# study-game-engines/directx-renderer-kurth

Measured on AMD Instinct MI355X. Metric: physics steps/sec at 100k rigid bodies, higher is better.
Workload: dtype f32; 1 GPU; c3: 100k mixed colliders (sphere/capsule/OBB), dt 1/120 s, 30 solver iterations; bodies=100000, broadphase_pairs=611032, manifolds=251275, contacts=317267, joints=0, recoveries=0, parallelism=1 gpu

## Files before the change

directx-renderer-kurth_amd/csrc/cluster.h:

```cpp
#pragma once
#include "world.h"

#define CL_TASKS_PER_PHASE 2u
#define CL_SUBCOUNTERS 8u
#define CL_LOCAL_STATIC 0xFFFFu
#define CL_SERIAL_COLOR 64u

MI_DEV u32 clHash(u32 x) { x ^= x >> 16; x *= 0x7feb352du; x ^= x >> 15; x *= 0x846ca68bu; x ^= x >> 16; return x; }
MI_DEV u32 clPhaseOffset(const u32* counters, u32 p)
{
	u32 off = p ? counters[CTR_CL_NUM_TASKS] : 0u;
	for (u32 q = CL_MAX_PHASES - 1u; q > p && p; --q) off += counters[CTR_CL_NUM_TASKS + q];
	return off;
}
struct ClTask
{
	u32 first, count, numBodies, numShared, numColors, serialStart, numRows, sharedBase;
	u32 colorStart[72];
};
static_assert(sizeof(ClTask) == 320, "task header");

bool cluster_color_setup(World& w, u32 computeUnits);
void cluster_color_launch(World& w, u32 nj);
u32 cluster_solve_setup(const World& w);
```

directx-renderer-kurth_amd/csrc/k_cluster_solve.hip:

```cpp
#include "cluster.h"
#include "solver_rows.h"
#include "joint_solve.h"

#define CL_MAX_LOCAL_TASKS 8u
#define CLS_LANES 512u
#define CLQ_QUADS (CLS_LANES / 4u)
#define CLQ_SETS 7u
#define CLQ_REG_CONTACTS (CLQ_QUADS * CLQ_SETS)
#define CLQ_SETS_JOINTS 4u
#define CL_SPIN_LIMIT (1u << 22)

typedef u32 u32x4 __attribute__((ext_vector_type(4)));

struct QuadRow { V3 dT, aT, dN, aN; float mT, mN, bias, friction, lamN, lamT; };
#define CLQ_ZERO_FLOAT4S (2u * CLQ_QUADS + 4u)
#define CLQ_ROW_FLOAT4S 14u

struct ClLocal
{
	u32 first, count, numBodies, numShared, numColors, serialStart, numContacts, phase, key, sharedBase, numJoints;
	u32 bodyOff;
	u32 infoOff;
	u32 regContacts, spill, rowOff, rowCap, scratchBase;
	u32 ldsColors;
	u32 colorStart[68];
};

struct ClArgs
{
	u32* counters; const ClTask* tasks; const u32* bodyList; const u32* phaseMask; const u32* sharedSlot;
	const u32* mKeySorted; const u32* mLocal; const u32* cEntry;
	const float4* rowPlanes; const float4* rowShared; float2* rowLambda; float4* rowScratch; u32 scratchContacts;
	u32 regContactsCap;
	u32 ldsRowsCap;
	u32 predictDiv, pollSleep;
	float4* vel; u64* flow; u64* trace;
	size_t rowCap; u32 nb, flowBytes, epoch, itBegin, itEnd, ldsFloat4s;
	const u32* jointClassStart; const uint2* taskJoints; const uint4* jointTable; float* jointUpd[MI_JOINT_TYPES]; const float4* invIw; u32 numJointClasses;
};

MI_DEV float clQuadSum(float p)
{
	float q = p + __builtin_bit_cast(float, __builtin_amdgcn_update_dpp(0, __builtin_bit_cast(int, p), 0xB1, 0xF, 0xF, false));
	return q + __builtin_bit_cast(float, __builtin_amdgcn_update_dpp(0, __builtin_bit_cast(int, q), 0x4E, 0xF, 0xF, false));
}
MI_DEV void clSolveQuad(QuadRow& r, V3& x)
{
	float vt = clQuadSum(rowDot3(x, r.dT));
	float maxFriction = r.friction * r.lamN;
	float newT = rowClampSym(__builtin_fmaf(-r.mT, vt, r.lamT), maxFriction);
	float d = newT - r.lamT; r.lamT = newT;
	x = rowFma(d, r.aT, x);
	float vn = clQuadSum(rowDot3(x, r.dN));
	float newN = fmaxf(__builtin_fmaf(-r.mN, vn - r.bias, r.lamN), 0.f);
	d = newN - r.lamN; r.lamN = newN;
	x = rowFma(d, r.aN, x);
}
MI_DEV void clBuildQuadRow(QuadRow& r, u32& addr, const ClLocal& L, const ClArgs& A, const float4* lds, u32 p, u32 q, u32 zeroRec, u32& slotOut, u32& kOut)
{
	const u32 e = A.cEntry[(size_t)4u * L.first + p], mp = e & 0xFFFu, k = e >> 12, slot = L.first + mp;
	const u32 ab = A.mLocal[slot], local = q < 2u ? (ab & 0xFFFFu) : (ab >> 16);
	const float4 sh = A.rowShared[slot];
	ContactRow row; loadRow(row, k, slot, A.rowCap, A.rowPlanes, A.rowLambda);
	const bool isStatic = local == CL_LOCAL_STATIC;
	addr = (isStatic ? zeroRec : L.bodyOff + 2u * local) + (q & 1u);
	const float invMass = isStatic ? 0.f : lds[L.bodyOff + 2u * local].w;
	const V3 t = v3(row.p0.x, row.p0.y, row.p0.z), n = v3(sh.x, sh.y, sh.z);
	if (q == 0u) { r.dT = -t; r.aT = -(invMass * t); r.dN = -n; r.aN = -(invMass * n); }
	else if (q == 1u) { r.dT = -v3(row.p0.w, row.p1.x, row.p1.y); r.aT = -v3(row.p3.w, row.p4.x, row.p4.y); r.dN = -v3(row.p2.y, row.p2.z, row.p2.w); r.aN = -v3(row.p5.y, row.p5.z, row.p5.w); }
	else if (q == 2u) { r.dT = t; r.aT = invMass * t; r.dN = n; r.aN = invMass * n; }
	else { r.dT = v3(row.p1.z, row.p1.w, row.p2.x); r.aT = v3(row.p4.z, row.p4.w, row.p5.x); r.dN = v3(row.p3.x, row.p3.y, row.p3.z); r.aN = v3(row.p6.x, row.p6.y, row.p6.z); }
	r.mT = row.p7.x; r.mN = row.p6.w; r.bias = row.p7.y; r.friction = sh.w; r.lamN = row.lam.x; r.lamT = row.lam.y;
	slotOut = slot; kOut = k;
}
template <typename T> MI_DEV T clLdsAt(const float4* lds, u32 byte) { return *(const T*)((const char*)lds + byte); }
template <typename PTR> MI_DEV void clStoreQuadRow(PTR P, u32 q, const QuadRow& r, u32 addr)
{
	P[3u * q] = make_float4(r.dT.x, r.dT.y, r.dT.z, r.aT.x); P[3u * q + 1u] = make_float4(r.aT.y, r.aT.z, r.dN.x, r.dN.y); P[3u * q + 2u] = make_float4(r.dN.z, r.aN.x, r.aN.y, r.aN.z);
	if (q == 0u) P[12] = make_float4(r.mT, r.mN, r.bias, r.friction);
	const u32 other = (u32)__builtin_amdgcn_update_dpp(0, (int)addr, 0xB1, 0xF, 0xF, false);
	const u32 otherPair = (u32)__builtin_amdgcn_update_dpp(0, (int)(addr | (other << 16)), 0x4E, 0xF, 0xF, false);
	if (q == 0u) P[13] = make_float4(r.lamN, r.lamT, __uint_as_float(addr | (other << 16)), __uint_as_float(otherPair));
}
MI_DEV u32 clPairAddr(u32 pair, u32 q) { return (q & 1u) ? (pair >> 16) : (pair & 0xFFFFu); }
#define CLQ_PAIR_WORD(q) (54u + ((q) >> 1))
template <typename PTR> MI_DEV void clLoadQuadRow(QuadRow& r, u32& addr, PTR P, u32 q)
{
	float4 a = P[3u * q], b = P[3u * q + 1u], c = P[3u * q + 2u], d = P[12], e = P[13];
	r.dT = v3f4(a); r.aT = v3(a.w, b.x, b.y); r.dN = v3(b.z, b.w, c.x); r.aN = v3(c.y, c.z, c.w);
	r.mT = d.x; r.mN = d.y; r.bias = d.z; r.friction = d.w; r.lamN = e.x; r.lamT = e.y;
	addr = clPairAddr(__float_as_uint(q < 2u ? e.z : e.w), q);
}

template <bool JOINTS> __global__ void __launch_bounds__(CLS_LANES) k_cl_solve(ClArgs A)
{
	extern __shared__ float4 lds[];
	__shared__ ClLocal sTask[CL_MAX_LOCAL_TASKS];
	__shared__ u32 sNumTasks, sAbort;
	__shared__ u32 sRegStart[CL_SERIAL_COLOR + 4u];
	const u32 tid = threadIdx.x, G = gridDim.x, quad = tid >> 2, q = tid & 3u;
	constexpr u32 SETS = JOINTS ? CLQ_SETS_JOINTS : CLQ_SETS;
	u32* status = A.counters + CTR_FLOW_STATUS;
	__amdgpu_buffer_rsrc_t rsrc = __builtin_amdgcn_make_buffer_rsrc(A.flow, 0, A.flowBytes, 0x00020000);
	const u32 zeroBase = A.ldsFloat4s - CLQ_ZERO_FLOAT4S, zeroRec = zeroBase + 2u * CLQ_QUADS, sinkRec = zeroRec + 2u;

	if (tid == 0)
	{
		if (A.trace) A.trace[(size_t)blockIdx.x * CL_TRACE_ROWS * CL_TRACE_WORDS + 15 * 32] = wall_clock64();
		u32 nT = 0, off = 0, used = 0;
		bool bad = A.counters[CTR_CL_STATUS] != 0u;
		for (u32 p = 0; p < CL_MAX_PHASES; ++p)
		{
			u32 tasksInPhase = A.counters[CTR_CL_NUM_TASKS + p];
			if (tasksInPhase > CL_TASKS_PER_PHASE * G) { bad = true; atomicOr(status, 128u); }
			off = clPhaseOffset(A.counters, p);
			u32 t = (blockIdx.x + G - (off % G)) % G;
			for (; t < tasksInPhase && !bad; t += G)
			{
				u32 key = p * CL_MAX_TASKS + t;
				const ClTask* T = A.tasks + key;
				const u32 tj = (A.jointClassStart && p == 0u) ? A.jointClassStart[(size_t)key * (CL_MAX_JOINT_CLASSES + 2u) + CL_MAX_JOINT_CLASSES] : 0u;
				if (!T->count && !tj) continue;
				if (nT == CL_MAX_LOCAL_TASKS) { bad = true; atomicOr(status, 256u); break; }
				ClLocal& L = sTask[nT];
				L.first = T->first; L.count = T->count; L.numBodies = T->numBodies; L.numShared = T->numShared; L.numColors = T->numColors; L.serialStart = T->serialStart; L.numContacts = T->numRows;
				L.phase = p; L.key = key; L.sharedBase = T->sharedBase; L.numJoints = tj;
				if (tj > CLS_LANES || (tj && nT)) { bad = true; atomicOr(status, 2048u); }
				for (u32 c = 0; c <= CL_SERIAL_COLOR + 1u; ++c) L.colorStart[c] = T->colorStart[c];
				L.colorStart[CL_SERIAL_COLOR + 2u] = L.colorStart[CL_SERIAL_COLOR + 1u]; L.colorStart[CL_SERIAL_COLOR + 3u] = L.colorStart[CL_SERIAL_COLOR + 1u];
				L.bodyOff = used; used += 2u * L.numBodies;
				L.infoOff = used * 4u; used += (3u * L.numBodies + 3u) / 4u;
				L.regContacts = (nT == 0) ? min(L.numContacts, min(CLQ_QUADS * SETS, A.regContactsCap)) : 0u;
				L.rowOff = 0; L.rowCap = 0; L.spill = 0;
				const u32 regBase = L.numContacts - L.regContacts;
				L.ldsColors = 0; while (L.ldsColors < L.numColors && L.colorStart[L.ldsColors + 1u] <= regBase) ++L.ldsColors;
				if (nT == 0) for (u32 c = 0; c < CL_SERIAL_COLOR + 4u; ++c) sRegStart[c] = L.colorStart[c] - regBase;
				++nT;
			}
		}
		if (used + CLQ_ZERO_FLOAT4S > A.ldsFloat4s) { bad = true; atomicOr(status, 512u); }
		u32 ldsRowsLeft = A.ldsRowsCap;
		for (u32 k = 0; k < nT && !bad; ++k)
		{
			ClLocal& L = sTask[k];
			u32 want = L.numContacts - L.regContacts;
			u32 left = A.ldsFloat4s - used - CLQ_ZERO_FLOAT4S;
			u32 fit = min(left / CLQ_ROW_FLOAT4S, ldsRowsLeft);
			u32 cap = want < fit ? want : fit;
			L.rowOff = used; L.rowCap = cap; used += CLQ_ROW_FLOAT4S * cap; ldsRowsLeft -= cap; L.scratchBase = 0; L.spill = want - cap;
			if (want > cap) { L.scratchBase = atomicAdd(&A.counters[CTR_CL_SCRATCH], want - cap); if (L.scratchBase + (want - cap) > A.scratchContacts) { bad = true; atomicOr(status, 1024u); break; } }
		}
		if (bad) atomicOr(status, 64u);
		sNumTasks = nT; sAbort = (bad || __hip_atomic_load(status, __ATOMIC_RELAXED, __HIP_MEMORY_SCOPE_AGENT) != 0u) ? 1u : 0u;
	}
	__syncthreads();
	if (sAbort) return;
	const u32 numTasks = sNumTasks;
	if (!numTasks) return;

	for (u32 k = 0; k < numTasks; ++k)
	{
		const ClLocal& L = sTask[k];
		u32* info = (u32*)lds + L.infoOff;
		for (u32 l = tid; l < L.numBodies; l += CLS_LANES)
		{
			u32 g = A.bodyList[(size_t)L.key * CL_BODY_STRIDE + l];
			u32 pm = A.phaseMask[g];
			u32 deg = __popc(pm), rank = __popc(pm & ((1u << L.phase) - 1u));
			u32 below = pm & ((1u << L.phase) - 1u);
			u32 prev = below ? 31u - (u32)__clz(below) : 31u - (u32)__clz(pm);
			info[3 * l] = g; info[3 * l + 1] = deg | (rank << 8);
			info[3 * l + 2] = (l < L.numShared) ? A.sharedSlot[(size_t)prev * (A.nb + 1u) + g] : 0u;
			lds[L.bodyOff + 2 * l] = A.vel[2 * g]; lds[L.bodyOff + 2 * l + 1] = A.vel[2 * g + 1];
		}
	}
	for (u32 i = tid; i < CLQ_ZERO_FLOAT4S; i += CLS_LANES) lds[zeroBase + i] = make_float4(0.f, 0.f, 0.f, 0.f);
	__syncthreads();
	QuadRow rows[SETS]; u32 addr[SETS];
	{
		const ClLocal& L = sTask[0];
		const u32 regBase = L.numContacts - L.regContacts;
#pragma unroll
		for (u32 s = 0; s < SETS; ++s)
		{
			const u32 p = s * CLQ_QUADS + quad;
			rows[s].dT = rows[s].aT = rows[s].dN = rows[s].aN = v3(0.f, 0.f, 0.f); rows[s].mT = rows[s].mN = rows[s].bias = rows[s].friction = rows[s].lamN = rows[s].lamT = 0.f; addr[s] = sinkRec;
			if (p < L.regContacts) { u32 slot, kk; clBuildQuadRow(rows[s], addr[s], L, A, lds, regBase + p, q, zeroBase + 2u * quad, slot, kk); }
		}
	}
	for (u32 k = 0; k < numTasks; ++k)
	{
		const ClLocal& L = sTask[k];
		for (u32 p = quad; p < L.numContacts - L.regContacts; p += CLQ_QUADS)
		{
			QuadRow r; u32 a, slot, kk;
			clBuildQuadRow(r, a, L, A, lds, p, q, zeroBase + 2u * quad, slot, kk);
			if (p >= L.spill) clStoreQuadRow(lds + L.rowOff + (p - L.spill) * CLQ_ROW_FLOAT4S, q, r, a);
			else clStoreQuadRow(A.rowScratch + (size_t)(L.scratchBase + p) * CLQ_ROW_FLOAT4S, q, r, a);
		}
	}
	u32 tailStart0 = sTask[0].numColors, tailSet = 0, myTail = 255u;
	{
		const ClLocal& L = sTask[0];
		const u32 regBase = L.numContacts - L.regContacts, endPos = L.colorStart[L.numColors];
		if (L.numColors && endPos > regBase)
		{
			const u32 blk = (endPos - regBase - 1u) >> 4;
			while (tailStart0 > 0u && L.colorStart[tailStart0 - 1u] >= regBase && ((L.colorStart[tailStart0 - 1u] - regBase) >> 4) == blk) --tailStart0;
			if (L.numColors - tailStart0 < 2u) tailStart0 = L.numColors;
			else
			{
				tailSet = (L.colorStart[tailStart0] - regBase) / CLQ_QUADS;
				const u32 p = regBase + tailSet * CLQ_QUADS + quad;
				if (p >= L.colorStart[tailStart0] && p < endPos) { myTail = tailStart0; while (L.colorStart[myTail + 1u] <= p) ++myTail; }
			}
		}
		tailStart0 = __builtin_amdgcn_readfirstlane(tailStart0); tailSet = __builtin_amdgcn_readfirstlane(tailSet);
	}
	const u32 bodyOff0 = sTask[0].bodyOff;
	u32 jClass = 0xFFFFFFFFu, jType = 0, jA = 0, jB = 0, jRdA = zeroRec, jWrA = sinkRec, jRdB = zeroRec, jWrB = sinkRec; float* jRec = nullptr;
	const u32 numJoints0 = (JOINTS && sTask[0].phase == 0u) ? sTask[0].numJoints : 0u;
	if (JOINTS && tid < numJoints0)
	{
		const u32* cs = A.jointClassStart + (size_t)sTask[0].key * (CL_MAX_JOINT_CLASSES + 2u);
		uint2 e = A.taskJoints[cs[CL_MAX_JOINT_CLASSES + 1u] + tid];
		uint4 t4 = A.jointTable[e.x];
		jType = t4.x & 0xFFu; jClass = t4.x >> 8; jA = t4.z; jB = t4.w;
		jRec = A.jointUpd[jType] + (size_t)t4.y * jointUpdateFloats(jType);
		u32 la = e.y & 0xFFFFu, lb = e.y >> 16;
		if (la != CL_LOCAL_STATIC) { jRdA = bodyOff0 + 2u * la; jWrA = jRdA; }
		if (lb != CL_LOCAL_STATIC) { jRdB = bodyOff0 + 2u * lb; jWrB = jRdB; }
	}
	__syncthreads();
	u64* trace = A.trace ? A.trace + (size_t)blockIdx.x * CL_TRACE_ROWS * CL_TRACE_WORDS : nullptr;
	if (trace && tid == 0)
	{
		trace[15 * 32 + 1] = wall_clock64();
		for (u32 k = 0; k < numTasks && k < 5u; ++k) { trace[15 * 32 + 2 + 4 * k] = sTask[k].count; trace[15 * 32 + 3 + 4 * k] = sTask[k].numColors; trace[15 * 32 + 4 + 4 * k] = sTask[k].numShared; trace[15 * 32 + 5 + 4 * k] = sTask[k].phase | (sTask[k].numBodies << 8) | ((u64)sTask[k].numContacts << 32); trace[15 * 32 + 22 + k] = sTask[k].rowCap | ((u64)sTask[k].regContacts << 32); trace[15 * 32 + 27 + k] = sTask[k].spill | ((u64)(k == 0u ? sTask[0].numColors - tailStart0 : 0u) << 32); }
	}

#define CLQ_SOLVE_SET(S_, CS_, END_) if ((S_) < SETS) { const u32 pos = (S_) * CLQ_QUADS + quad; if (pos >= (CS_) && pos < (END_)) { float4 b = lds[addr[(S_) < SETS ? (S_) : 0u]]; V3 x = v3f4(b); clSolveQuad(rows[(S_) < SETS ? (S_) : 0u], x); lds[addr[(S_) < SETS ? (S_) : 0u]] = make_float4(x.x, x.y, x.z, b.w); } }
#define CLQ_PREFETCH(POS_) { const u32 in_ = max((POS_), spill) + quad - spill; if (in_ < rowCap) pfW = ((const u32*)(lds + rowOff + in_ * CLQ_ROW_FLOAT4S))[CLQ_PAIR_WORD(q)]; }
#define CLQ_SOLVE_ROWS(CS_, END_) \
	{ \
		u32 w = pfW; \
		CLQ_PREFETCH(END_) \
		for (u32 p = (CS_) + quad; p < (END_); p += CLQ_QUADS) \
		{ \
			const bool inLds = p >= spill; \
			QuadRow r; u32 a; float4 b; \
			float4* P = lds + rowOff + (inLds ? p - spill : 0u) * CLQ_ROW_FLOAT4S; \
			float4* S = A.rowScratch + (size_t)(scratchBase + (inLds ? 0u : p)) * CLQ_ROW_FLOAT4S; \
			u32 wn = 0u; if (p + CLQ_QUADS < (END_) && p + CLQ_QUADS >= spill) wn = ((const u32*)(lds + rowOff + (p + CLQ_QUADS - spill) * CLQ_ROW_FLOAT4S))[CLQ_PAIR_WORD(q)]; \
			if (inLds) { u32 unused; a = clPairAddr(w, q); b = lds[a]; clLoadQuadRow(r, unused, P, q); } else { clLoadQuadRow(r, a, S, q); b = lds[a]; } \
			V3 x = v3f4(b); clSolveQuad(r, x); lds[a] = make_float4(x.x, x.y, x.z, b.w); \
			if (q == 0u) { if (inLds) ((float2*)(P + 13))[0] = make_float2(r.lamN, r.lamT); else ((float2*)(S + 13))[0] = make_float2(r.lamN, r.lamT); } \
			w = wn; \
		} \
	}
#define CLQ_SOLVE_ROWS_LDS(CS_, END_) \
	{ \
		const u32 i = (CS_) - spill + quad, endR = (END_) - spill, w = pfW; \
		pfW = clLdsAt<u32>(lds, __umul24(min(endR + quad, lastRow), CLQ_ROW_FLOAT4S * 16u) + pairByte); \
		if (i < endR) \
		{ \
			const u32 a = clPairAddr(w, q), rowByte = __umul24(i, CLQ_ROW_FLOAT4S * 16u) + rowsByte, own = rowByte + q * 48u; \
			const float4 b = lds[a], r0 = clLdsAt<float4>(lds, own), r1 = clLdsAt<float4>(lds, own + 16u), r2 = clLdsAt<float4>(lds, own + 32u), r3 = clLdsAt<float4>(lds, rowByte + 192u); \
			const float2 lam = clLdsAt<float2>(lds, rowByte + 208u); \
			QuadRow r; r.dT = v3f4(r0); r.aT = v3(r0.w, r1.x, r1.y); r.dN = v3(r1.z, r1.w, r2.x); r.aN = v3(r2.y, r2.z, r2.w); \
			r.mT = r3.x; r.mN = r3.y; r.bias = r3.z; r.friction = r3.w; r.lamN = lam.x; r.lamT = lam.y; \
			V3 x = v3f4(b); clSolveQuad(r, x); lds[a] = make_float4(x.x, x.y, x.z, b.w); \
			if (q == 0u) *(float2*)((char*)lds + (rowByte + 208u)) = make_float2(r.lamN, r.lamT); \
		} \
	}
#define CLQ_ADVANCE(END_) \
	__syncthreads(); \
	if (stamp && c < 63u && (END_) == csNext) { trace[5 * 32 + 1 + c] = clock64(); trace[7 * 32 + c] = L.colorStart[c + 1u] - L.colorStart[c]; } \
	if ((END_) == csNext) { csCur = csNext; csNext = __builtin_amdgcn_readfirstlane(csAfter); ++c; } else csCur = (END_);
#define CLQ_SET_LOOP(S_) \
	if ((S_) < SETS) while (c < mainColors && csCur < min(regC, ((S_) + 1u) * CLQ_QUADS)) \
	{ \
// ... 93 lines not shown
			{
				const u32 numColors = __builtin_amdgcn_readfirstlane(L.numColors), serialStart = __builtin_amdgcn_readfirstlane(L.serialStart), numContacts = __builtin_amdgcn_readfirstlane(L.numContacts);
				const u32 regC = __builtin_amdgcn_readfirstlane(L.regContacts), rowOff = __builtin_amdgcn_readfirstlane(L.rowOff), rowCap = __builtin_amdgcn_readfirstlane(L.rowCap), scratchBase = __builtin_amdgcn_readfirstlane(L.scratchBase);
				const u32 spill = __builtin_amdgcn_readfirstlane(L.spill), ldsColors = __builtin_amdgcn_readfirstlane(L.ldsColors), regBase = numContacts - regC;
				const bool stamp = trace && tid == 0 && it == A.itBegin + 10u && k == 0;
				if (stamp) trace[5 * 32] = clock64();
				const u32 mainColors = (k == 0u) ? tailStart0 : numColors;
				u32 c = 0, csCur = __builtin_amdgcn_readfirstlane(L.colorStart[0]), csNext = __builtin_amdgcn_readfirstlane(L.colorStart[1]);
				if (__builtin_expect(regBase != 0u, 0))
				{
					while (c < mainColors && csCur < spill)
					{
						const u32 csAfter = L.colorStart[c + 2u];
						const u32 end = min(csNext, spill);
						CLQ_SOLVE_ROWS(csCur, end)
						CLQ_ADVANCE(end)
					}
					{
						const u32 rowsByte = rowOff * 16u, lastRow = max(rowCap, 1u) - 1u, pairByte = rowsByte + 4u * CLQ_PAIR_WORD(q);
						while (c < ldsColors)
						{
							const u32 csAfter = L.colorStart[c + 2u];
							const u32 end = min(csNext, csCur + CLQ_QUADS);
							CLQ_SOLVE_ROWS_LDS(csCur, end)
							CLQ_ADVANCE(end)
						}
						while (c < mainColors && csCur < regBase)
						{
							const u32 csAfter = L.colorStart[c + 2u];
							const u32 end = min(regBase, csCur + CLQ_QUADS);
							CLQ_SOLVE_ROWS_LDS(csCur, end)
							CLQ_ADVANCE(end)
						}
					}
					csCur -= regBase; csNext -= regBase;
				}
				CLQ_SET_LOOP(0) CLQ_SET_LOOP(1) CLQ_SET_LOOP(2) CLQ_SET_LOOP(3) CLQ_SET_LOOP(4) CLQ_SET_LOOP(5) CLQ_SET_LOOP(6) CLQ_SET_LOOP(7)
				if (mainColors < numColors)
				{
#define CLQ_TAIL(S_) case S_: if ((S_) < SETS && myTail != 255u) for (u32 ct = mainColors; ct < numColors; ++ct) { if (myTail == ct) { float4 b = lds[addr[(S_) < SETS ? (S_) : 0u]]; V3 x = v3f4(b); clSolveQuad(rows[(S_) < SETS ? (S_) : 0u], x); lds[addr[(S_) < SETS ? (S_) : 0u]] = make_float4(x.x, x.y, x.z, b.w); } __builtin_amdgcn_fence(__ATOMIC_ACQ_REL, "wavefront"); } break;
					switch (tailSet) { CLQ_TAIL(0) CLQ_TAIL(1) CLQ_TAIL(2) CLQ_TAIL(3) CLQ_TAIL(4) CLQ_TAIL(5) CLQ_TAIL(6) CLQ_TAIL(7) default: break; }
#undef CLQ_TAIL
					__syncthreads();
					if (stamp) for (u32 ct = mainColors; ct < numColors && ct < 63u; ++ct) { trace[5 * 32 + 1 + ct] = clock64(); trace[7 * 32 + ct] = L.colorStart[ct + 1u] - L.colorStart[ct]; }
				}
				if (serialStart < numContacts) CLQ_PREFETCH(serialStart)
				for (u32 sp = serialStart; sp < numContacts; ++sp)
				{
					if (sp >= regBase)
					{
						const u32 rp = sp - regBase;
						switch (rp / CLQ_QUADS)
						{
							case 0: CLQ_SOLVE_SET(0u, rp, rp + 1u) break; case 1: CLQ_SOLVE_SET(1u, rp, rp + 1u) break; case 2: CLQ_SOLVE_SET(2u, rp, rp + 1u) break; case 3: CLQ_SOLVE_SET(3u, rp, rp + 1u) break;
							case 4: CLQ_SOLVE_SET(4u, rp, rp + 1u) break; case 5: CLQ_SOLVE_SET(5u, rp, rp + 1u) break; case 6: CLQ_SOLVE_SET(6u, rp, rp + 1u) break; default: CLQ_SOLVE_SET(7u, rp, rp + 1u) break;
						}
					}
					else { CLQ_SOLVE_ROWS(sp, sp + 1u) }
					__syncthreads();
				}
			}
			if (trace && tid == 0 && it - A.itBegin < 32u && k < 5u) trace[(3 * k + 1) * 32 + (it - A.itBegin)] = wall_clock64();
			for (u32 l = tid; l < L.numShared; l += CLS_LANES)
			{
				u32 g = info[3 * l], ti = info[3 * l + 1];
				u32 deg = ti & 0xFFu, rank = ti >> 8;
				u32 want = A.epoch + (it - A.itBegin) * deg + rank;
				u32 rec = (L.sharedBase + l) * 32u;
				float4 b0 = lds[L.bodyOff + 2 * l], b1 = lds[L.bodyOff + 2 * l + 1];
				if (it + 1u == A.itEnd && rank + 1u == deg) { A.vel[2 * g] = b0; A.vel[2 * g + 1] = make_float4(b1.x, b1.y, b1.z, 0.f); }
				else
				{
					u32x4 h1 = { __float_as_uint(b1.x), __float_as_uint(b1.y), __float_as_uint(b1.z), want + 1u };
					u32x4 h0 = { __float_as_uint(b0.x), __float_as_uint(b0.y), __float_as_uint(b0.z), want + 1u };
					__builtin_amdgcn_raw_buffer_store_b128(h1, rsrc, rec + 16u, 0, 16);
					__builtin_amdgcn_raw_buffer_store_b128(h0, rsrc, rec, 0, 16);
				}
			}
			if (k + 1u == numTasks) lastPublish = wall_clock64();
			CLQ_PREFETCH_TURN(k + 1u < numTasks ? k + 1u : 0u)
		}
	}
	if (aborted) return;

	for (u32 k = 0; k < numTasks; ++k)
	{
		const ClLocal& L = sTask[k];
		const u32* info = (const u32*)lds + L.infoOff;
		for (u32 l = L.numShared + tid; l < L.numBodies; l += CLS_LANES)
		{
			u32 g = info[3 * l];
			float4 b1 = lds[L.bodyOff + 2 * l + 1];
			A.vel[2 * g] = lds[L.bodyOff + 2 * l]; A.vel[2 * g + 1] = make_float4(b1.x, b1.y, b1.z, 0.f);
		}
		if (q == 0u)
		{
			if (k == 0)
			{
#pragma unroll
				for (u32 s = 0; s < SETS; ++s)
				{
					const u32 p = s * CLQ_QUADS + quad;
					if (p < L.regContacts) { const u32 e = A.cEntry[(size_t)4u * L.first + (L.numContacts - L.regContacts) + p]; A.rowLambda[(size_t)(e >> 12) * A.rowCap + L.first + (e & 0xFFFu)] = make_float2(rows[s].lamN, rows[s].lamT); }
				}
			}
			for (u32 p = quad; p < L.numContacts - L.regContacts; p += CLQ_QUADS)
			{
				const u32 e = A.cEntry[(size_t)4u * L.first + p];
				const float4 lam = p >= L.spill ? lds[L.rowOff + (p - L.spill) * CLQ_ROW_FLOAT4S + 13u] : A.rowScratch[(size_t)(L.scratchBase + p) * CLQ_ROW_FLOAT4S + 13u];
				A.rowLambda[(size_t)(e >> 12) * A.rowCap + L.first + (e & 0xFFFu)] = make_float2(lam.x, lam.y);
			}
		}
	}
#undef CLQ_SET_LOOP
#undef CLQ_ADVANCE
#undef CLQ_SOLVE_ROWS
#undef CLQ_SOLVE_ROWS_LDS
#undef CLQ_PREFETCH
#undef CLQ_PREFETCH_TURN
#undef CLQ_SOLVE_SET
}

bool cluster_solves_joints(const World& w) { return w.cluster.jointsInCluster && w.cluster.jointsEnabled; }

u32 cluster_solve_setup(const World& w)
{
	int maxLds = 0;
	MI_CHECK(hipDeviceGetAttribute(&maxLds, hipDeviceAttributeMaxSharedMemoryPerBlock, w.device));
	hipFuncAttributes fa = {};
	MI_CHECK(hipFuncGetAttributes(&fa, (const void*)k_cl_solve<true>));
	size_t dyn = (maxLds > 0 ? (size_t)maxLds : 65536) - fa.sharedSizeBytes - 256;
	dyn &= ~(size_t)15;
	if (hipFuncSetAttribute((const void*)k_cl_solve<false>, hipFuncAttributeMaxDynamicSharedMemorySize, (int)dyn) != hipSuccess
		|| hipFuncSetAttribute((const void*)k_cl_solve<true>, hipFuncAttributeMaxDynamicSharedMemorySize, (int)dyn) != hipSuccess) return 0u;
	return (u32)dyn;
}

bool cluster_available(World& w)
{
	if (w.cluster.ldsBytes) return w.cluster.ldsBytes != ~0u;
	int cus = 0;
	MI_CHECK(hipDeviceGetAttribute(&cus, hipDeviceAttributeMultiprocessorCount, w.device));
	const u32 dyn = cluster_solve_setup(w);
	if (!dyn || !cluster_color_setup(w, (u32)std::max(1, cus)))
	{
		(void)hipGetLastError();
		w.cluster.ldsBytes = ~0u;
		return false;
	}
	w.cluster.ldsBytes = dyn; w.cluster.blocks = (u32)std::max(1, cus);
	if (w.cluster.blocksLimit) w.cluster.blocks = std::min(w.cluster.blocks, w.cluster.blocksLimit);
	return true;
}

static const u32 CL_PREDICT_DIV = 4;
static const u32 CL_POLL_SLEEP = 1;

void launch_cluster_solve(World& w, u32 itBegin, u32 itEnd)
{
	if (itBegin >= itEnd) return;
	size_t words = (size_t)(w.nb + 1) * CL_MAX_PHASES * 4;
	if (w.cluster.flow.cap < words) { w.cluster.flow.ensure(words, w.stream); w.cluster.flowEpoch = 0; if (w.lastError) return; }
	if (w.cluster.flowEpoch == 0 || w.cluster.flowEpoch >= 0xFFFEu)
	{
		MI_CHECK(hipMemsetAsync(w.cluster.flow.p, 0, sizeof(u64) * words, w.stream));
		w.cluster.flowEpoch = 0;
	}
	w.cluster.flowEpoch++;
	if (w.cluster.flowTestAbortStep == w.stats.numInternalSteps)
	{
		u32 one = 16u;
		MI_CHECK(hipMemcpyAsync(w.dCounters.p + CTR_FLOW_STATUS, &one, sizeof(u32), hipMemcpyHostToDevice, w.stream));
		MI_CHECK(hipStreamSynchronize(w.stream));
	}
	const size_t scratchContacts = std::min<size_t>(2 * w.pairCap, 512u * 1024u);
	w.cluster.rowScratch.ensure(scratchContacts * CLQ_ROW_FLOAT4S, w.stream);
	if (w.lastError) return;
	if (itBegin) MI_CHECK(hipMemsetAsync(w.dCounters.p + CTR_CL_SCRATCH, 0, sizeof(u32), w.stream));
	ClArgs A;
	A.rowScratch = w.cluster.rowScratch.p; A.scratchContacts = (u32)scratchContacts; A.regContactsCap = w.cluster.regContactsCap; A.ldsRowsCap = w.cluster.ldsRowsCap;
	A.counters = w.dCounters.p; A.tasks = (const ClTask*)w.cluster.tasks.p; A.bodyList = w.cluster.bodyList.p; A.phaseMask = w.cluster.phaseMask.p; A.sharedSlot = w.cluster.sharedSlot.p;
	A.mKeySorted = w.mKeySorted.p; A.mLocal = w.cluster.local.p; A.cEntry = w.cluster.entry.p;
	A.rowPlanes = w.rowPlanes.p; A.rowShared = w.rowShared.p; A.rowLambda = w.rowLambda.p; A.vel = w.vel.p; A.flow = w.cluster.flow.p; A.trace = w.cluster.flowTrace.p; A.predictDiv = CL_PREDICT_DIV; A.pollSleep = CL_POLL_SLEEP;
	A.rowCap = w.rowCap; A.nb = w.nb; A.flowBytes = (u32)(words * sizeof(u64)); A.epoch = w.cluster.flowEpoch << 16; A.itBegin = itBegin; A.itEnd = itEnd;
	A.ldsFloat4s = w.cluster.ldsBytes / 16u;
	const bool withJoints = cluster_solves_joints(w);
	A.jointClassStart = withJoints ? w.cluster.jointClassStart.p : nullptr; A.taskJoints = w.cluster.taskJoints.p; A.jointTable = w.cluster.jointTable.p; A.invIw = w.invIw.p; A.numJointClasses = withJoints ? w.cluster.numJointClasses : 0u;
	for (u32 t = 0; t < MI_JOINT_TYPES; ++t) A.jointUpd[t] = w.joints[t].dUpdate.p;
	if (withJoints) hipLaunchKernelGGL(k_cl_solve<true>, dim3(w.cluster.blocks), dim3(CLS_LANES), w.cluster.ldsBytes, w.stream, A);
	else hipLaunchKernelGGL(k_cl_solve<false>, dim3(w.cluster.blocks), dim3(CLS_LANES), w.cluster.ldsBytes, w.stream, A);
}
```

Baseline: 627.3 steps/s.

## Parallelise cluster-solve launch head and batch row fetches ahead of use

The serial single-thread task-header scan in the cluster solve kernel becomes a cooperative staging step. All lanes copy candidate task headers into LDS, a shared host/device layout routine computes the local layout, and then 64 lanes per task fill the per-task color tables. Contact-row construction and the final lambda write-back now issue batched, prefetched global loads (fetch-ahead for register rows, batches of 2/4 for LDS rows), so several loads are in flight instead of dependent one-by-one loads. This adds LDS staging requirements and extra trace stamps, and the layout logic is duplicated into a new header with static_asserts.

```diff
diff --git a/directx-renderer-kurth_amd/csrc/cluster.h b/directx-renderer-kurth_amd/csrc/cluster.h
--- a/directx-renderer-kurth_amd/csrc/cluster.h
+++ b/directx-renderer-kurth_amd/csrc/cluster.h
@@ -1,7 +1,7 @@
 #pragma once
 #include "world.h"
 
-#define CL_TASKS_PER_PHASE 2u
+#include "cluster_layout.h"
 #define CL_SUBCOUNTERS 8u
 #define CL_LOCAL_STATIC 0xFFFFu
 #define CL_SERIAL_COLOR 64u
@@ -19,6 +19,9 @@
 	u32 colorStart[72];
 };
 static_assert(sizeof(ClTask) == 320, "task header");
+static_assert(sizeof(ClTask) == 4u * CL_HDR_WORDS && offsetof(ClTask, count) == 4u * CL_HDR_COUNT && offsetof(ClTask, numBodies) == 4u * CL_HDR_NUM_BODIES && offsetof(ClTask, numColors) == 4u * CL_HDR_NUM_COLORS
+	&& offsetof(ClTask, numRows) == 4u * CL_HDR_NUM_ROWS && offsetof(ClTask, colorStart) == 4u * CL_HDR_COLOR_START, "cluster_layout.h: the header's words");
+static_assert(CL_LAYOUT_PHASES == CL_MAX_PHASES && CL_LAYOUT_COLORS == CL_SERIAL_COLOR, "cluster_layout.h: the limits");
 
 bool cluster_color_setup(World& w, u32 computeUnits);
 void cluster_color_launch(World& w, u32 nj);
diff --git a/directx-renderer-kurth_amd/csrc/cluster_layout.h b/directx-renderer-kurth_amd/csrc/cluster_layout.h
--- /dev/null
+++ b/directx-renderer-kurth_amd/csrc/cluster_layout.h
@@ -0,0 +1,100 @@
+#pragma once
+#include <stdint.h>
+#if defined(__HIPCC__)
+#define CL_LAYOUT_FN __host__ __device__ inline
+#else
+#define CL_LAYOUT_FN inline
+#endif
+
+#define CL_TASKS_PER_PHASE 2u
+#define CL_MAX_LOCAL_TASKS 8u
+#define CL_LAYOUT_PHASES 5u
+#define CL_LAYOUT_CANDIDATES (CL_TASKS_PER_PHASE * CL_LAYOUT_PHASES)
+#define CL_LAYOUT_COLORS 64u
+#define CL_HDR_WORDS 80u
+#define CL_HDR_COUNT 1u
+#define CL_HDR_NUM_BODIES 2u
+#define CL_HDR_NUM_COLORS 4u
+#define CL_HDR_NUM_ROWS 6u
+#define CL_HDR_COLOR_START 8u
+#define CL_GIVE_UP 64u
+#define CL_GIVE_UP_PHASE_TASKS 128u
+#define CL_GIVE_UP_LOCAL_TASKS 256u
+#define CL_GIVE_UP_BODIES 512u
+#define CL_GIVE_UP_SCRATCH 1024u
+#define CL_GIVE_UP_JOINTS 2048u
+
+struct ClLayoutParams
+{
+	uint32_t buildStatus;
+	uint32_t G, block;
+	uint32_t regContactsMax;
+	uint32_t ldsRowsCap;
+	uint32_t ldsFloat4s, zeroFloat4s, rowFloat4s;
+	uint32_t maxJoints;
+};
+struct ClLayoutOut
+{
+	uint32_t numTasks, status, bad;
+	uint32_t cand[CL_MAX_LOCAL_TASKS], phase[CL_MAX_LOCAL_TASKS], task[CL_MAX_LOCAL_TASKS], numJoints[CL_MAX_LOCAL_TASKS];
+	uint32_t bodyOff[CL_MAX_LOCAL_TASKS], infoOff[CL_MAX_LOCAL_TASKS];
+	uint32_t regContacts[CL_MAX_LOCAL_TASKS], ldsColors[CL_MAX_LOCAL_TASKS];
+	uint32_t rowOff[CL_MAX_LOCAL_TASKS], rowCap[CL_MAX_LOCAL_TASKS], spill[CL_MAX_LOCAL_TASKS];
+	uint32_t numRequests, requestTask[CL_MAX_LOCAL_TASKS];
+};
+
+CL_LAYOUT_FN uint32_t clLayoutPhaseOffset(const uint32_t* tasksInPhase, uint32_t p)
+{
+	uint32_t off = p ? tasksInPhase[0] : 0u;
+	for (uint32_t q = CL_LAYOUT_PHASES - 1u; q > p && p; --q) off += tasksInPhase[q];
+	return off;
+}
+CL_LAYOUT_FN uint32_t clLayoutFirstTask(const uint32_t* tasksInPhase, uint32_t G, uint32_t block, uint32_t p)
+{
+	return (block + G - (clLayoutPhaseOffset(tasksInPhase, p) % G)) % G;
+}
+
+CL_LAYOUT_FN void clLayout(const ClLayoutParams& P, const uint32_t* tasksInPhase, const uint32_t* hdr, const uint32_t* numJoints, ClLayoutOut& o)
+{
+	uint32_t nT = 0, used = 0, status = 0;
+	bool bad = P.buildStatus != 0u;
+	for (uint32_t p = 0; p < CL_LAYOUT_PHASES; ++p)
+	{
+		const uint32_t n = tasksInPhase[p];
+		if (n > CL_TASKS_PER_PHASE * P.G) { bad = true; status |= CL_GIVE_UP_PHASE_TASKS; }
+		uint32_t t = clLayoutFirstTask(tasksInPhase, P.G, P.block, p);
+		for (uint32_t j = 0; t < n && !bad; t += P.G, ++j)
+		{
+			const uint32_t c = p * CL_TASKS_PER_PHASE + j;
+			const uint32_t* H = hdr + c * CL_HDR_WORDS;
+			const uint32_t tj = numJoints[c];
+			if (!H[CL_HDR_COUNT] && !tj) continue;
+			if (nT == CL_MAX_LOCAL_TASKS) { bad = true; status |= CL_GIVE_UP_LOCAL_TASKS; break; }
+			o.cand[nT] = c; o.phase[nT] = p; o.task[nT] = t; o.numJoints[nT] = tj;
+			if (tj > P.maxJoints || (tj && nT)) { bad = true; status |= CL_GIVE_UP_JOINTS; }
+			const uint32_t numBodies = H[CL_HDR_NUM_BODIES], numContacts = H[CL_HDR_NUM_ROWS], numColors = H[CL_HDR_NUM_COLORS];
+			o.bodyOff[nT] = used; used += 2u * numBodies;
+			o.infoOff[nT] = used * 4u; used += (3u * numBodies + 3u) / 4u;
+			const uint32_t regContacts = (nT == 0u) ? (numContacts < P.regContactsMax ? numContacts : P.regContactsMax) : 0u;
+			o.regContacts[nT] = regContacts; o.rowOff[nT] = 0; o.rowCap[nT] = 0; o.spill[nT] = 0;
+			const uint32_t regBase = numContacts - regContacts;
+			uint32_t ldsColors = 0, open = 1u;
+			for (uint32_t k = 0; k < numColors && k < CL_LAYOUT_COLORS + 1u; ++k) { open &= (H[CL_HDR_COLOR_START + k + 1u] <= regBase) ? 1u : 0u; ldsColors += open; }
+			o.ldsColors[nT] = ldsColors;
+			++nT;
+		}
+	}
+	if (used + P.zeroFloat4s > P.ldsFloat4s) { bad = true; status |= CL_GIVE_UP_BODIES; }
+	uint32_t ldsRowsLeft = P.ldsRowsCap, numRequests = 0;
+	for (uint32_t k = 0; k < nT && !bad; ++k)
+	{
+		const uint32_t numContacts = hdr[o.cand[k] * CL_HDR_WORDS + CL_HDR_NUM_ROWS];
+		const uint32_t want = numContacts - o.regContacts[k];
+		const uint32_t left = P.ldsFloat4s - used - P.zeroFloat4s;
+		const uint32_t byLds = left / P.rowFloat4s, fit = byLds < ldsRowsLeft ? byLds : ldsRowsLeft;
+		const uint32_t cap = want < fit ? want : fit;
+		o.rowOff[k] = used; o.rowCap[k] = cap; used += P.rowFloat4s * cap; ldsRowsLeft -= cap; o.spill[k] = want - cap;
+		if (want > cap) o.requestTask[numRequests++] = k;
+	}
+	o.numTasks = nT; o.numRequests = numRequests; o.status = status; o.bad = bad ? 1u : 0u;
+}
diff --git a/directx-renderer-kurth_amd/csrc/k_cluster_solve.hip b/directx-renderer-kurth_amd/csrc/k_cluster_solve.hip
--- a/directx-renderer-kurth_amd/csrc/k_cluster_solve.hip
+++ b/directx-renderer-kurth_amd/csrc/k_cluster_solve.hip
@@ -2,18 +2,24 @@
 #include "solver_rows.h"
 #include "joint_solve.h"
 
-#define CL_MAX_LOCAL_TASKS 8u
+#define CL_STAGE_LAYOUT_WORD 832u
+#define CL_STAGE_BYTES 4096u
 #define CLS_LANES 512u
 #define CLQ_QUADS (CLS_LANES / 4u)
 #define CLQ_SETS 7u
 #define CLQ_REG_CONTACTS (CLQ_QUADS * CLQ_SETS)
 #define CLQ_SETS_JOINTS 4u
+#define CLQ_FETCH_AHEAD 3u
+#define CLQ_BUILD_BATCH 2u
+#define CLQ_HOME_BATCH 4u
+#define CL_TRACE_ROW_HEAD 2u
 #define CL_SPIN_LIMIT (1u << 22)
 
 typedef u32 u32x4 __attribute__((ext_vector_type(4)));
 
 struct QuadRow { V3 dT, aT, dN, aN; float mT, mN, bias, friction, lamN, lamT; };
 #define CLQ_ZERO_FLOAT4S (2u * CLQ_QUADS + 4u)
+static_assert(4u * CL_STAGE_LAYOUT_WORD >= 4u * (CL_LAYOUT_CANDIDATES * CL_HDR_WORDS + CL_LAYOUT_CANDIDATES + CL_LAYOUT_PHASES) && 4u * CL_STAGE_LAYOUT_WORD + sizeof(ClLayoutOut) <= CL_STAGE_BYTES && CL_STAGE_LAYOUT_WORD % 4u == 0u, "the launch head's staging area");
 #define CLQ_ROW_FLOAT4S 14u
 
 struct ClLocal
@@ -56,22 +62,30 @@
 	d = newN - r.lamN; r.lamN = newN;
 	x = rowFma(d, r.aN, x);
 }
-MI_DEV void clBuildQuadRow(QuadRow& r, u32& addr, const ClLocal& L, const ClArgs& A, const float4* lds, u32 p, u32 q, u32 zeroRec, u32& slotOut, u32& kOut)
-{
-	const u32 e = A.cEntry[(size_t)4u * L.first + p], mp = e & 0xFFFu, k = e >> 12, slot = L.first + mp;
-	const u32 ab = A.mLocal[slot], local = q < 2u ? (ab & 0xFFFFu) : (ab >> 16);
-	const float4 sh = A.rowShared[slot];
-	ContactRow row; loadRow(row, k, slot, A.rowCap, A.rowPlanes, A.rowLambda);
+__device__ __forceinline__ void clAllIn(u32 (&e)[2]) { asm volatile("" : "+v"(e[0]), "+v"(e[1])); }
+__device__ __forceinline__ void clAllIn(u32 (&e)[4]) { asm volatile("" : "+v"(e[0]), "+v"(e[1]), "+v"(e[2]), "+v"(e[3])); }
+__device__ __forceinline__ void clAllIn(u32 (&e)[7]) { asm volatile("" : "+v"(e[0]), "+v"(e[1]), "+v"(e[2]), "+v"(e[3]), "+v"(e[4]), "+v"(e[5]), "+v"(e[6])); }
+struct ClRawRow { ContactRow row; float4 sh; u32 ab; };
+MI_DEV void clFetchRow(ClRawRow& f, u32 first, const ClArgs& A, u32 e)
+{
+	const u32 slot = first + (e & 0xFFFu);
+	f.ab = A.mLocal[slot]; f.sh = A.rowShared[slot];
+	loadRow(f.row, e >> 12, slot, A.rowCap, A.rowPlanes, A.rowLambda);
+}
+MI_DEV void clFinishQuadRow(QuadRow& r, u32& addr, const ClRawRow& f, u32 bodyOff, const float4* lds, u32 q, u32 zeroRec)
+{
+	const ContactRow& row = f.row; const float4 sh = f.sh;
+	const u32 local = q < 2u ? (f.ab & 0xFFFFu) : (f.ab >> 16);
 	const bool isStatic = local == CL_LOCAL_STATIC;
-	addr = (isStatic ? zeroRec : L.bodyOff + 2u * local) + (q & 1u);
-	const float invMass = isStatic ? 0.f : lds[L.bodyOff + 2u * local].w;
+	const u32 body = isStatic ? zeroRec : bodyOff + 2u * local;
+	addr = body + (q & 1u);
+	const float invMass = isStatic ? 0.f : lds[body].w;
 	const V3 t = v3(row.p0.x, row.p0.y, row.p0.z), n = v3(sh.x, sh.y, sh.z);
 	if (q == 0u) { r.dT = -t; r.aT = -(invMass * t); r.dN = -n; r.aN = -(invMass * n); }
 	else if (q == 1u) { r.dT = -v3(row.p0.w, row.p1.x, row.p1.y); r.aT = -v3(row.p3.w, row.p4.x, row.p4.y); r.dN = -v3(row.p2.y, row.p2.z, row.p2.w); r.aN = -v3(row.p5.y, row.p5.z, row.p5.w); }
 	else if (q == 2u) { r.dT = t; r.aT = invMass * t; r.dN = n; r.aN = invMass * n; }
 	else { r.dT = v3(row.p1.z, row.p1.w, row.p2.x); r.aT = v3(row.p4.z, row.p4.w, row.p5.x); r.dN = v3(row.p3.x, row.p3.y, row.p3.z); r.aN = v3(row.p6.x, row.p6.y, row.p6.z); }
 	r.mT = row.p7.x; r.mN = row.p6.w; r.bias = row.p7.y; r.friction = sh.w; r.lamN = row.lam.x; r.lamT = row.lam.y;
-	slotOut = slot; kOut = k;
 }
 template <typename T> MI_DEV T clLdsAt(const float4* lds, u32 byte) { return *(const T*)((const char*)lds + byte); }
 template <typename PTR> MI_DEV void clStoreQuadRow(PTR P, u32 q, const QuadRow& r, u32 addr)
@@ -96,7 +110,7 @@
 {
 	extern __shared__ float4 lds[];
 	__shared__ ClLocal sTask[CL_MAX_LOCAL_TASKS];
-	__shared__ u32 sNumTasks, sAbort;
+	__shared__ u32 sNumTasks, sAbort, sGaveUp;
 	__shared__ u32 sRegStart[CL_SERIAL_COLOR + 4u];
 	const u32 tid = threadIdx.x, G = gridDim.x, quad = tid >> 2, q = tid & 3u;
 	constexpr u32 SETS = JOINTS ? CLQ_SETS_JOINTS : CLQ_SETS;
@@ -104,60 +118,84 @@
 	__amdgpu_buffer_rsrc_t rsrc = __builtin_amdgcn_make_buffer_rsrc(A.flow, 0, A.flowBytes, 0x00020000);
 	const u32 zeroBase = A.ldsFloat4s - CLQ_ZERO_FLOAT4S, zeroRec = zeroBase + 2u * CLQ_QUADS, sinkRec = zeroRec + 2u;
 
+	u32* const stage = (u32*)lds;
+	u32* const stageJoints = stage + CL_LAYOUT_CANDIDATES * CL_HDR_WORDS;
+	u32* const stageCounts = stageJoints + CL_LAYOUT_CANDIDATES;
+	ClLayoutOut& lay = *(ClLayoutOut*)(stage + CL_STAGE_LAYOUT_WORD);
+	if (tid == 0 && A.trace) A.trace[(size_t)blockIdx.x * CL_TRACE_ROWS * CL_TRACE_WORDS + 15 * 32] = wall_clock64();
+	const u32 buildStatus = A.counters[CTR_CL_STATUS];
+	{
+		u32 cnt[CL_MAX_PHASES];
+#pragma unroll
+		for (u32 pp = 0; pp < CL_MAX_PHASES; ++pp) cnt[pp] = A.counters[CTR_CL_NUM_TASKS + pp];
+		const u32 p = tid >> 6, j = (tid >> 5) & 1u, word = tid & 31u, c = p * CL_TASKS_PER_PHASE + j;
+		u32 n = 0, first = 0;
+#pragma unroll
+		for (u32 pp = 0; pp < CL_MAX_PHASES; ++pp) if (pp == p) { n = cnt[pp]; first = clLayoutFirstTask(cnt, G, blockIdx.x, pp); }
+		if (p < CL_MAX_PHASES)
+		{
+			const u32 t = first + j * G, key = p * CL_MAX_TASKS + t;
+			const bool have = t < n && t < CL_MAX_TASKS;
+			if (word < CL_HDR_WORDS / 4u) { uint4 h = make_uint4(0u, 0u, 0u, 0u); if (have) h = ((const uint4*)(A.tasks + key))[word]; ((uint4*)stage)[c * (CL_HDR_WORDS / 4u) + word] = h; }
+			else if (word == CL_HDR_WORDS / 4u) { u32 tj = 0u; if (have && p == 0u && A.jointClassStart) tj = A.jointClassStart[(size_t)key * (CL_MAX_JOINT_CLASSES + 2u) + CL_MAX_JOINT_CLASSES]; stageJoints[c] = tj; }
+			else if (word == CL_HDR_WORDS / 4u + 1u && j == 0u) stageCounts[p] = n;
+		}
+	}
+	__syncthreads();
 	if (tid == 0)
 	{
-		if (A.trace) A.trace[(size_t)blockIdx.x * CL_TRACE_ROWS * CL_TRACE_WORDS + 15 * 32] = wall_clock64();
-		u32 nT = 0, off = 0, used = 0;
-		bool bad = A.counters[CTR_CL_STATUS] != 0u;
-		for (u32 p = 0; p < CL_MAX_PHASES; ++p)
-		{
-			u32 tasksInPhase = A.counters[CTR_CL_NUM_TASKS + p];
-			if (tasksInPhase > CL_TASKS_PER_PHASE * G) { bad = true; atomicOr(status, 128u); }
-			off = clPhaseOffset(A.counters, p);
-			u32 t = (blockIdx.x + G - (off % G)) % G;
-			for (; t < tasksInPhase && !bad; t += G)
-			{
-				u32 key = p * CL_MAX_TASKS + t;
-				const ClTask* T = A.tasks + key;
-				const u32 tj = (A.jointClassStart && p == 0u) ? A.jointClassStart[(size_t)key * (CL_MAX_JOINT_CLASSES + 2u) + CL_MAX_JOINT_CLASSES] : 0u;
-				if (!T->count && !tj) continue;
-				if (nT == CL_MAX_LOCAL_TASKS) { bad = true; atomicOr(status, 256u); break; }
-				ClLocal& L = sTask[nT];
-				L.first = T->first; L.count = T->count; L.numBodies = T->numBodies; L.numShared = T->numShared; L.numColors = T->numColors; L.serialStart = T->serialStart; L.numContacts = T->numRows;
-				L.phase = p; L.key = key; L.sharedBase = T->sharedBase; L.numJoints = tj;
-				if (tj > CLS_LANES || (tj && nT)) { bad = true; atomicOr(status, 2048u); }
-				for (u32 c = 0; c <= CL_SERIAL_COLOR + 1u; ++c) L.colorStart[c] = T->colorStart[c];
-				L.colorStart[CL_SERIAL_COLOR + 2u] = L.colorStart[CL_SERIAL_COLOR + 1u]; L.colorStart[CL_SERIAL_COLOR + 3u] = L.colorStart[CL_SERIAL_COLOR + 1u];
-				L.bodyOff = used; used += 2u * L.numBodies;
-				L.infoOff = used * 4u; used += (3u * L.numBodies + 3u) / 4u;
-				L.regContacts = (nT == 0) ? min(L.numContacts, min(CLQ_QUADS * SETS, A.regContactsCap)) : 0u;
-				L.rowOff = 0; L.rowCap = 0; L.spill = 0;
-				const u32 regBase = L.numContacts - L.regContacts;
-				L.ldsColors = 0; while (L.ldsColors < L.numColors && L.colorStart[L.ldsColors + 1u] <= regBase) ++L.ldsColors;
-				if (nT == 0) for (u32 c = 0; c < CL_SERIAL_COLOR + 4u; ++c) sRegStart[c] = L.colorStart[c] - regBase;
-				++nT;
-			}
-		}
-		if (used + CLQ_ZERO_FLOAT4S > A.ldsFloat4s) { bad = true; atomicOr(status, 512u); }
-		u32 ldsRowsLeft = A.ldsRowsCap;
-		for (u32 k = 0; k < nT && !bad; ++k)
-		{
+		ClLayoutParams P;
+		P.buildStatus = buildStatus; P.G = G; P.block = blockIdx.x; P.regContactsMax = min(CLQ_QUADS * SETS, A.regContactsCap); P.ldsRowsCap = A.ldsRowsCap;
+		P.ldsFloat4s = A.ldsFloat4s; P.zeroFloat4s = CLQ_ZERO_FLOAT4S; P.rowFloat4s = CLQ_ROW_FLOAT4S; P.maxJoints = CLS_LANES;
+		clLayout(P, stageCounts, stage, stageJoints, lay);
+		u32 giveUp = lay.status; bool bad = lay.bad != 0u;
+		for (u32 k = 0; k < lay.numTasks; ++k) sTask[k].scratchBase = 0;
+		for (u32 r = 0; r < lay.numRequests && !bad; ++r)
+		{
+			const u32 k = lay.requestTask[r], rows = lay.spill[k], base = atomicAdd(&A.counters[CTR_CL_SCRATCH], rows);
+			sTask[k].scratchBase = base;
+			if (base + rows > A.scratchContacts) { bad = true; giveUp |= CL_GIVE_UP_SCRATCH; }
+		}
+		if (bad) giveUp |= CL_GIVE_UP;
+		if (giveUp) atomicOr(status, giveUp);
+		sNumTasks = lay.numTasks; sAbort = bad ? 1u : 0u;
+	}
+	else if (tid == CLS_LANES - 64u) sGaveUp = __hip_atomic_load(status, __ATOMIC_RELAXED, __HIP_MEMORY_SCOPE_AGENT);
+	__syncthreads();
+	{
+		const u32 k = tid >> 6, l = tid & 63u;
+		if (k < sNumTasks)
+		{
+			const u32* H = stage + lay.cand[k] * CL_HDR_WORDS;
 			ClLocal& L = sTask[k];
-			u32 want = L.numContacts - L.regContacts;
-			u32 left = A.ldsFloat4s - used - CLQ_ZERO_FLOAT4S;
-			u32 fit = min(left / CLQ_ROW_FLOAT4S, ldsRowsLeft);
-			u32 cap = want < fit ? want : fit;
-			L.rowOff = used; L.rowCap = cap; used += CLQ_ROW_FLOAT4S * cap; ldsRowsLeft -= cap; L.scratchBase = 0; L.spill = want - cap;
-			if (want > cap) { L.scratchBase = atomicAdd(&A.counters[CTR_CL_SCRATCH], want - cap); if (L.scratchBase + (want - cap) > A.scratchContacts) { bad = true; atomicOr(status, 1024u); break; } }
-		}
-		if (bad) atomicOr(status, 64u);
-		sNumTasks = nT; sAbort = (bad || __hip_atomic_load(status, __ATOMIC_RELAXED, __HIP_MEMORY_SCOPE_AGENT) != 0u) ? 1u : 0u;
+			const u32 regBase = H[CL_HDR_NUM_ROWS] - lay.regContacts[k];
+			const u32 cs = H[CL_HDR_COLOR_START + l], csEnd = H[CL_HDR_COLOR_START + CL_SERIAL_COLOR + min(l, 1u)];
+			L.colorStart[l] = cs; if (l < 4u) L.colorStart[CL_SERIAL_COLOR + l] = csEnd;
+			if (k == 0u) { sRegStart[l] = cs - regBase; if (l < 4u) sRegStart[CL_SERIAL_COLOR + l] = csEnd - regBase; }
+			if (l == 0u)
+			{
+				L.first = H[0]; L.count = H[CL_HDR_COUNT]; L.numBodies = H[CL_HDR_NUM_BODIES]; L.numShared = H[3]; L.numColors = H[CL_HDR_NUM_COLORS]; L.serialStart = H[5]; L.numContacts = H[CL_HDR_NUM_ROWS]; L.sharedBase = H[7];
+				L.phase = lay.phase[k]; L.key = lay.phase[k] * CL_MAX_TASKS + lay.task[k]; L.numJoints = lay.numJoints[k];
+				L.bodyOff = lay.bodyOff[k]; L.infoOff = lay.infoOff[k]; L.regContacts = lay.regContacts[k]; L.ldsColors = lay.ldsColors[k];
+				L.rowOff = lay.rowOff[k]; L.rowCap = lay.rowCap[k]; L.spill = lay.spill[k];
+			}
+		}
 	}
 	__syncthreads();
-	if (sAbort) return;
+	if (A.trace && tid == 0) A.trace[((size_t)blockIdx.x * CL_TRACE_ROWS + CL_TRACE_ROW_HEAD) * CL_TRACE_WORDS] = wall_clock64();
+	if (sAbort | sGaveUp) return;
 	const u32 numTasks = sNumTasks;
 	if (!numTasks) return;
 
+	const u32 regC0 = __builtin_amdgcn_readfirstlane(sTask[0].regContacts), first0 = __builtin_amdgcn_readfirstlane(sTask[0].first);
+	u32 eReg[SETS]; ClRawRow fReg[CLQ_FETCH_AHEAD];
+	{
+		const u32* entry = A.cEntry + (size_t)4u * first0 + (sTask[0].numContacts - regC0);
+#pragma unroll
+		for (u32 s = 0; s < SETS; ++s) { eReg[s] = 0u; if (s * CLQ_QUADS < regC0) eReg[s] = entry[min(s * CLQ_QUADS + quad, regC0 - 1u)]; }
+#pragma unroll
+		for (u32 s = 0; s < CLQ_FETCH_AHEAD && s < SETS; ++s) if (s * CLQ_QUADS < regC0) clFetchRow(fReg[s], first0, A, eReg[s]);
+	}
 	for (u32 k = 0; k < numTasks; ++k)
 	{
 		const ClLocal& L = sTask[k];
@@ -166,37 +204,58 @@
 		{
 			u32 g = A.bodyList[(size_t)L.key * CL_BODY_STRIDE + l];
 			u32 pm = A.phaseMask[g];
+			const float4 v0 = A.vel[2 * g], v1 = A.vel[2 * g + 1];
 			u32 deg = __popc(pm), rank = __popc(pm & ((1u << L.phase) - 1u));
 			u32 below = pm & ((1u << L.phase) - 1u);
 			u32 prev = below ? 31u - (u32)__clz(below) : 31u - (u32)__clz(pm);
 			info[3 * l] = g; info[3 * l + 1] = deg | (rank << 8);
 			info[3 * l + 2] = (l < L.numShared) ? A.sharedSlot[(size_t)prev * (A.nb + 1u) + g] : 0u;
-			lds[L.bodyOff + 2 * l] = A.vel[2 * g]; lds[L.bodyOff + 2 * l + 1] = A.vel[2 * g + 1];
+			lds[L.bodyOff + 2 * l] = v0; lds[L.bodyOff + 2 * l + 1] = v1;
 		}
 	}
 	for (u32 i = tid; i < CLQ_ZERO_FLOAT4S; i += CLS_LANES) lds[zeroBase + i] = make_float4(0.f, 0.f, 0.f, 0.f);
 	__syncthreads();
+	if (A.trace && tid == 0) A.trace[((size_t)blockIdx.x * CL_TRACE_ROWS + CL_TRACE_ROW_HEAD) * CL_TRACE_WORDS + 1] = wall_clock64();
 	QuadRow rows[SETS]; u32 addr[SETS];
 	{
-		const ClLocal& L = sTask[0];
-		const u32 regBase = L.numContacts - L.regContacts;
+		const u32 bodyOff = sTask[0].bodyOff;
 #pragma unroll
 		for (u32 s = 0; s < SETS; ++s)
 		{
-			const u32 p = s * CLQ_QUADS + quad;
 			rows[s].dT = rows[s].aT = rows[s].dN = rows[s].aN = v3(0.f, 0.f, 0.f); rows[s].mT = rows[s].mN = rows[s].bias = rows[s].friction = rows[s].lamN = rows[s].lamT = 0.f; addr[s] = sinkRec;
-			if (p < L.regContacts) { u32 slot, kk; clBuildQuadRow(rows[s], addr[s], L, A, lds, regBase + p, q, zeroBase + 2u * quad, slot, kk); }
-		}
-	}
+			if (s * CLQ_QUADS < regC0)
+			{
+				QuadRow r; u32 a;
+				clFinishQuadRow(r, a, fReg[s % CLQ_FETCH_AHEAD], bodyOff, lds, q, zeroBase + 2u * quad);
+				if (s + CLQ_FETCH_AHEAD < SETS && (s + CLQ_FETCH_AHEAD) * CLQ_QUADS < regC0) clFetchRow(fReg[s % CLQ_FETCH_AHEAD], first0, A, eReg[(s + CLQ_FETCH_AHEAD) % SETS]);
+				if (s * CLQ_QUADS + quad < regC0) { rows[s] = r; addr[s] = a; }
+			}
+		}
+	}
+	if (A.trace && tid == 0) A.trace[((size_t)blockIdx.x * CL_TRACE_ROWS + CL_TRACE_ROW_HEAD) * CL_TRACE_WORDS + 2] = wall_clock64();
 	for (u32 k = 0; k < numTasks; ++k)
 	{
 		const ClLocal& L = sTask[k];
-		for (u32 p = quad; p < L.numContacts - L.regContacts; p += CLQ_QUADS)
-		{
-			QuadRow r; u32 a, slot, kk;
-			clBuildQuadRow(r, a, L, A, lds, p, q, zeroBase + 2u * quad, slot, kk);
-			if (p >= L.spill) clStoreQuadRow(lds + L.rowOff + (p - L.spill) * CLQ_ROW_FLOAT4S, q, r, a);
-			else clStoreQuadRow(A.rowScratch + (size_t)(L.scratchBase + p) * CLQ_ROW_FLOAT4S, q, r, a);
+		const u32 below = L.numContacts - L.regContacts, first = L.first, bodyOff = L.bodyOff;
+		const u32* entry = A.cEntry + (size_t)4u * first;
+		for (u32 base = 0; base < below; base += CLQ_BUILD_BATCH * CLQ_QUADS)
+		{
+			u32 e[CLQ_BUILD_BATCH]; ClRawRow f[CLQ_BUILD_BATCH];
+#pragma unroll
+			for (u32 b = 0; b < CLQ_BUILD_BATCH; ++b) e[b] = entry[min(base + b * CLQ_QUADS + quad, below - 1u)];
+			clAllIn(e);
+#pragma unroll
+			for (u32 b = 0; b < CLQ_BUILD_BATCH; ++b) clFetchRow(f[b], first, A, e[b]);
+#pragma unroll
+			for (u32 b = 0; b < CLQ_BUILD_BATCH; ++b)
+			{
+				const u32 p = base + b * CLQ_QUADS + quad;
+				QuadRow r; u32 a;
+				clFinishQuadRow(r, a, f[b], bodyOff, lds, q, zeroBase + 2u * quad);
+				if (p >= below) continue;
+				if (p >= L.spill) clStoreQuadRow(lds + L.rowOff + (p - L.spill) * CLQ_ROW_FLOAT4S, q, r, a);
+				else clStoreQuadRow(A.rowScratch + (size_t)(L.scratchBase + p) * CLQ_ROW_FLOAT4S, q, r, a);
+			}
 		}
 	}
 	u32 tailStart0 = sTask[0].numColors, tailSet = 0, myTail = 255u;
@@ -456,6 +515,7 @@
 		}
 	}
 	if (aborted) return;
+	if (trace && tid == 0) trace[CL_TRACE_ROW_HEAD * 32 + 3] = lastPublish;
 
 	for (u32 k = 0; k < numTasks; ++k)
 	{
@@ -469,23 +529,36 @@
 		}
 		if (q == 0u)
 		{
-			if (k == 0)
-			{
+			const u32* entry = A.cEntry + (size_t)4u * L.first;
+			const u32 below = L.numContacts - L.regContacts;
+			if (k == 0 && L.regContacts)
+			{
+				u32 e[SETS];
+#pragma unroll
+				for (u32 s = 0; s < SETS; ++s) e[s] = entry[below + min(s * CLQ_QUADS + quad, L.regContacts - 1u)];
+				clAllIn(e);
 #pragma unroll
 				for (u32 s = 0; s < SETS; ++s)
-				{
-					const u32 p = s * CLQ_QUADS + quad;
-					if (p < L.regContacts) { const u32 e = A.cEntry[(size_t)4u * L.first + (L.numContacts - L.regContacts) + p]; A.rowLambda[(size_t)(e >> 12) * A.rowCap + L.first + (e & 0xFFFu)] = make_float2(rows[s].lamN, rows[s].lamT); }
-				}
-			}
-			for (u32 p = quad; p < L.numContacts - L.regContacts; p += CLQ_QUADS)
-			{
-				const u32 e = A.cEntry[(size_t)4u * L.first + p];
-				const float4 lam = p >= L.spill ? lds[L.rowOff + (p - L.spill) * CLQ_ROW_FLOAT4S + 13u] : A.rowScratch[(size_t)(L.scratchBase + p) * CLQ_ROW_FLOAT4S + 13u];
-				A.rowLambda[(size_t)(e >> 12) * A.rowCap + L.first + (e & 0xFFFu)] = make_float2(lam.x, lam.y);
-			}
-		}
-	}
+					if (s * CLQ_QUADS + quad < L.regContacts) A.rowLambda[(size_t)(e[s] >> 12) * A.rowCap + L.first + (e[s] & 0xFFFu)] = make_float2(rows[s].lamN, rows[s].lamT);
+			}
+			for (u32 base = 0; base < below; base += CLQ_HOME_BATCH * CLQ_QUADS)
+			{
+				u32 e[CLQ_HOME_BATCH];
+#pragma unroll
+				for (u32 b = 0; b < CLQ_HOME_BATCH; ++b) e[b] = entry[min(base + b * CLQ_QUADS + quad, below - 1u)];
+				clAllIn(e);
+#pragma unroll
+				for (u32 b = 0; b < CLQ_HOME_BATCH; ++b)
+				{
+					const u32 p = base + b * CLQ_QUADS + quad;
+					if (p >= below) continue;
+					const float4 lam = p >= L.spill ? lds[L.rowOff + (p - L.spill) * CLQ_ROW_FLOAT4S + 13u] : A.rowScratch[(size_t)(L.scratchBase + p) * CLQ_ROW_FLOAT4S + 13u];
+					A.rowLambda[(size_t)(e[b] >> 12) * A.rowCap + L.first + (e[b] & 0xFFFu)] = make_float2(lam.x, lam.y);
+				}
+			}
+		}
+	}
+	if (trace) { __syncthreads(); if (tid == 0) trace[CL_TRACE_ROW_HEAD * 32 + 4] = wall_clock64(); }
 #undef CLQ_SET_LOOP
 #undef CLQ_ADVANCE
 #undef CLQ_SOLVE_ROWS
@@ -505,6 +578,7 @@
 	MI_CHECK(hipFuncGetAttributes(&fa, (const void*)k_cl_solve<true>));
 	size_t dyn = (maxLds > 0 ? (size_t)maxLds : 65536) - fa.sharedSizeBytes - 256;
 	dyn &= ~(size_t)15;
+	if (dyn < CL_STAGE_BYTES + 16u * CLQ_ZERO_FLOAT4S) return 0u;
 	if (hipFuncSetAttribute((const void*)k_cl_solve<false>, hipFuncAttributeMaxDynamicSharedMemorySize, (int)dyn) != hipSuccess
 		|| hipFuncSetAttribute((const void*)k_cl_solve<true>, hipFuncAttributeMaxDynamicSharedMemorySize, (int)dyn) != hipSuccess) return 0u;
 	return (u32)dyn;
```

After: 629.9 steps/s, median of 6. No clear change (+0.4%).
